# qurator-spk/sbb_textline_detection

Measured on AMD Instinct MI355X. Metric: segmented patches/sec (448x448x3) per GPU + per-pixel label-map match vs ref, higher is better.
Workload: dtype f16x3; 1 GPU; BASELINE configs[1] x 32: 32 pages of 3500x2500 (70 tiles of 448x448 each, margin 0.1) per GPU per step, textline model, 2 classes; workload_id=page, dedupe=False, max_batch=320, lanes=2, owned_regions=1, exchange=none

## Files before the change

sbb_textline_detection_amd/csrc/api.hip:

```cpp
#include <stdarg.h>
#include <stdio.h>
#include <stdlib.h>
#include <string.h>

#include <algorithm>
#include <cmath>
#include <new>
#include <stdexcept>
#include <string>
#include <utility>
#include <vector>

#include "../../include/sbbseg.h"
#include <dlfcn.h>

#include <mutex>

#include "internal.h"
#include "region.h"
#include "profile_stat.h"
#include "line_mask.h"
#include "line_split.h"

using namespace sbbseg;
// ... 139 lines not shown
    double prof_ms = 0;
    int64_t prof_launches = 0, prof_patches = 0;
    int region_level = -1;
    double exec_patches = 0;
    double prof_exec_patches = 0;
};

struct PendingEvent { int op; hipEvent_t a, b; int patches; double exec; };

struct RegionRun {
    bool on = false;
    int kind[kRegionMaxLevels] = {0};
    int total[kRegionMaxLevels] = {0};
    double frac[kRegionMaxLevels] = {0};
    uint32_t* tab[kRegionMaxLevels] = {nullptr};
};

}

struct sbbseg_ctx {
    int device = 0;
    int precision = kBF16;
    int elem = 2;
    int planes = 1;
    hipStream_t own_stream = nullptr;
    hipStream_t stream = nullptr;
    hipStream_t lane_stream = nullptr;
    hipEvent_t ev_fork = nullptr, ev_join = nullptr;
    int lanes = 2, lane1_batch = 0;
    int lane_prio = 0, prio_least = 0, prio_greatest = 0;
// ... 63 lines not shown
    bool block_pq = true;
    bool unfuse_blocks = false;
    bool unfuse_stem_pool = false;
    bool no_dec_halo = false;
    bool no_expand_reduce = false;
    bool no_c3er = false;
    bool plain_gather = false;
    int contig_max_k = 0;
    int fused_heads = 0;
    int num_cus = 256;
    std::vector<PendingEvent> pending;
    std::vector<hipEvent_t> free_events;
    int owned_mode = 1;
    int region_levels = 0;
    int region_op[kRegionMaxLevels] = {0};
    uint32_t* d_rtab[2][kRegionMaxLevels] = {{nullptr}, {nullptr}};
    size_t rtab_cap[2][kRegionMaxLevels] = {{0}, {0}};
    RegionRun rr;
    double last_exec_frac = 1.0;
    std::vector<std::pair<void*, size_t>> user_bufs;
};

namespace {

int dmalloc(sbbseg_ctx* c, void** p, size_t bytes)
{
    HIPCHK(hipMalloc(p, bytes));
    c->device_bytes += bytes;
    return 0;
}
// ... 177 lines not shown
            if (rlv >= 0 && c->rr.kind[rlv] == 1) {
                if (p.fast_gather && !p.half_stages && p.variant != 2 && !(p.variant_flags & 4)) { p.rmap = c->rr.tab[rlv]; p.M = c->rr.total[rlv]; }
                else c->last_exec_frac = 1.0;
            }
            if (co.d_stem_wfrag && !(c->conv_variant & 3)) {
                const Tensor& st = c->tensors[co.d.src[0].tensor];
                StemParams sp;
                sp.pairs = st.buf; sp.PHt = st.H; sp.PWt = st.W; sp.n = n; sp.Ho = co.Ho; sp.Wo = co.Wo;
                sp.wfrag = co.d_stem_wfrag; sp.scale = co.d_scale; sp.shift = co.d_shift; sp.relu = co.d.relu; sp.wmul = co.wmul_cls[0];
                sp.out = c->tensors[co.d.out_tensor].data();
                if (co.fused_pool >= 0 && !c->unfuse_stem_pool) {
                    const PoolOp& po = c->ops[co.fused_pool].pool;
                    sp.pool_out = c->tensors[po.dst].data(); sp.pool_scale = po.d_pre_scale; sp.pool_shift = po.d_pre_shift;
                    sp.pool_relu = po.pre_relu; sp.pool_Ho = po.Ho; sp.pool_Wo = po.Wo;
                    sp.x3 = c->precision == kF16X3;
                    HIPCHK(launch_stem_pool_x3(sp, c->num_cus, c->stream));
                } else
                    HIPCHK(launch_stem(sp, c->precision, c->num_cus, c->stream));
            } else if (co.d_d64_wfrag && !(c->conv_variant & 3)) {
                const Tensor& st = c->tensors[co.d.src[0].tensor];
                Direct64Params dp;
                dp.src = st.buf; dp.n = n; dp.H = st.H; dp.W = st.W; dp.wfrag = co.d_d64_wfrag;
                dp.scale = co.d_scale; dp.shift = co.d_shift; dp.relu = co.d.relu; dp.out = c->tensors[co.d.out_tensor].data();
                dp.wmul = co.wmul_cls[0];
                HIPCHK(launch_direct64(dp, c->precision, c->num_cus, c->stream));
            } else if (co.fused_reduce >= 0 && !c->no_expand_reduce && !(c->conv_variant & 3)) {
                const ConvOp& ro = c->ops[co.fused_reduce].conv;
                if (co.fused_conv3 >= 0 && !c->no_c3er) {
                    const ConvOp& k3 = c->ops[co.fused_conv3].conv;
                    const Tensor& ta = c->tensors[k3.d.src[0].tensor];
// ... 52 lines not shown
            }
        } else if (op.type == kPool) {
            const PoolOp& po = op.pool;
            if (po.fused_into_stem && !c->unfuse_stem_pool && !(c->conv_variant & 3)) return 0;
            const Tensor& s = c->tensors[po.src];
            HIPCHK(launch_maxpool(s.data(), c->tensors[po.dst].data(), n, s.H, s.W, s.C, po.k, po.stride, po.Ho, po.Wo,
                                  po.d_pre_scale, po.d_pre_shift, po.pre_relu, c->precision, c->stream));
        } else if (op.type == kTail) {
            const TailOp& to = op.tail;
            const Tensor& s0 = c->tensors[to.src0];
            TailParams tp;
            tp.src0 = s0.buf; tp.img = c->tensors[to.img].buf; tp.PH = s0.H; tp.PW = s0.W; tp.n = n;
            tp.wfrag = to.d_wfrag; tp.scale = to.d_scale; tp.shift = to.d_shift; tp.classes = to.classes;
            tp.head_w = to.d_head_w; tp.head_scale = to.d_head_scale; tp.head_shift = to.d_head_shift;
            tp.labels = d_labels; tp.probs = d_probs;
            if (c->rr.on && op.region_level >= 0) {
                if (c->rr.total[op.region_level] == 0) return 0;
                tp.ttab = c->rr.tab[op.region_level]; tp.n_tab = c->rr.total[op.region_level];
            }
            HIPCHK(launch_tail(tp, c->precision, c->num_cus, c->stream));
        } else {
            const HeadOp& ho = op.head;
            const Tensor& s = c->tensors[ho.src];
            HeadParams hp;
            hp.src = s.data(); hp.cin = ho.cin; hp.classes = ho.classes; hp.M = n * s.H * s.W;
            hp.w = ho.d_w; hp.scale = ho.d_scale; hp.shift = ho.d_shift;
            hp.labels = d_labels; hp.probs = d_probs;
            HIPCHK(launch_head(hp, c->precision, c->stream));
        }
    return 0;
// ... 294 lines not shown
        (void)hipFree(c->pp_d_in[k]); (void)hipFree(c->pp_d_out[k]); (void)hipFree(c->pp_d_out3[k]);
        if (c->pp_in[k]) (void)hipEventDestroy(c->pp_in[k]);
        if (c->pp_comp[k]) (void)hipEventDestroy(c->pp_comp[k]);
        if (c->pp_out[k]) (void)hipEventDestroy(c->pp_out[k]);
    }
    comm_release(c);
    if (c->copy_in) (void)hipStreamDestroy(c->copy_in);
    if (c->copy_out) (void)hipStreamDestroy(c->copy_out);
    (void)hipFree(c->d_morph_a); (void)hipFree(c->d_morph_b); (void)hipFree(c->d_cc_parent); (void)hipFree(c->d_cc_count); (void)hipFree(c->d_cc_aux); (void)hipFree(c->d_cc_list); (void)hipFree(c->d_cc_small);
    for (auto& pe : c->pending) { (void)hipEventDestroy(pe.a); (void)hipEventDestroy(pe.b); }
    for (auto e : c->free_events) (void)hipEventDestroy(e);
    if (c->own_stream) (void)hipStreamDestroy(c->own_stream);
    if (c->lane_stream) (void)hipStreamDestroy(c->lane_stream);
    if (c->ev_fork) (void)hipEventDestroy(c->ev_fork);
    if (c->ev_join) (void)hipEventDestroy(c->ev_join);
    delete c;
    return 0;
    API_END
}

int sbbseg_set_stream(sbbseg_ctx* c, void* hip_stream)
{
    API_BEGIN
    REQUIRE(c, "null handle");
    if (resolve_pending(c)) return 1;
    c->stream = hip_stream == SBBSEG_OWN_STREAM ? c->own_stream : (hipStream_t)hip_stream;
    int up = 0;
    if (hip_stream != SBBSEG_OWN_STREAM && hip_stream && c->lane_prio != 0 && c->prio_least != c->prio_greatest &&
        hipStreamGetPriority((hipStream_t)hip_stream, &up) == hipSuccess && up == c->lane_prio) {
        const int other = c->lane_prio == c->prio_greatest ? c->prio_least : c->prio_greatest;
// ... 1090 lines not shown
            Op& b = c->ops[i + 1];
            if (a.type != kConv || !a.conv.d_stem_wfrag || b.type != kPool) continue;
            const PoolOp& po = b.pool;
            const Tensor& f1 = c->tensors[a.conv.d.out_tensor];
            if (po.src != a.conv.d.out_tensor || po.k != 3 || po.stride != 2 || !po.d_pre_scale || f1.C != 64 || (f1.H & 15) || (f1.W & 15) ||
                po.Ho != f1.H / 2 - 1 || po.Wo != f1.W / 2 - 1)
                continue;
            a.conv.fused_pool = (int)(i + 1);
            b.pool.fused_into_stem = true;
        }
    }
    REQUIRE(max_batch >= 1, "max_batch must be >= 1");
    REQUIRE(c->classes > 0 && !c->ops.empty(), "plan must contain a head (head op or a conv with a fused head)");
    c->max_batch = max_batch;
    find_region_chain(c);
    for (auto& t : c->tensors) {
        const size_t bytes = kZeroHeaderBytes + t.elems_per_patch * max_batch * c->elem * c->planes + 256;
        REQUIRE(bytes < ((size_t)1 << 32), "tensor %dx%dx%d x batch %d exceeds the 4 GiB gather window", t.H, t.W, t.C, max_batch);
        if (dmalloc(c, (void**)&t.lane_buf[0], bytes)) return 1;
        t.buf = t.lane_buf[0];
        HIPCHK(hipMemset(t.buf, 0, t.is_input_form ? bytes : (size_t)kZeroHeaderBytes));
    }
    c->lane1_batch = (c->lanes == 2 && max_batch >= 2 * kMinLaneTiles) ? (max_batch + 1) / 2 : 0;
    if (c->lane1_batch)
        for (auto& t : c->tensors) {
            const size_t bytes = kZeroHeaderBytes + t.elems_per_patch * c->lane1_batch * c->elem * c->planes + 256;
            if (dmalloc(c, (void**)&t.lane_buf[1], bytes)) return 1;
            HIPCHK(hipMemset(t.lane_buf[1], 0, t.is_input_form ? bytes : (size_t)kZeroHeaderBytes));
        }
    for (const Op& op : c->ops)
// ... 163 lines not shown
{
    REQUIRE(d_pages && n_pages >= 1 && d_tile_labels && first_tile >= 0 && n_tiles >= 0, "bad arguments");
    for (int k = 0; k < n_pages; ++k) REQUIRE(d_pages[k], "null page pointer (page %d)", k);
    int nx = 0, ny = 0;
    if (fused_grid(c, Hp, Wp, dedupe, &nx, &ny)) return 1;
    const int tpp = nx * ny;
    REQUIRE((long)first_tile + n_tiles <= (long)tpp * n_pages, "tile range [%d,%d) exceeds the %d tiles of the %d page(s)", first_tile,
            first_tile + n_tiles, tpp * n_pages, n_pages);
    const int margin = margin_of(c->in_W);
    IngestParams ip;
    if (fill_ingest(c, ip)) return 1;
    ip.page = (const uint8_t*)d_pages[0]; ip.Hp = Hp; ip.Wp = Wp; ip.src_Hp = src_Hp; ip.src_Wp = src_Wp; ip.tile_xy = nullptr;
    ip.map_y = d_map_y; ip.map_x = d_map_x; ip.bin_thr = d_bin_thr;
    ip.grid_nyf = ny; ip.grid_mid_x = c->in_W - 2 * margin; ip.grid_mid_y = c->in_H - 2 * margin;
    const size_t per = (size_t)c->in_H * c->in_W;
    const size_t act = (size_t)c->elem * c->planes;
    const bool regions = owned && c->region_levels > 0 && c->max_batch <= kRegionMaxPatches;
    RegionGeom rg;
    memset(&rg, 0, sizeof(rg));
    if (regions) {
        rg.ax = {Wp, c->in_W, margin, c->in_W - 2 * margin, nx};
        rg.ay = {Hp, c->in_H, margin, c->in_H - 2 * margin, ny};
        rg.tpp = tpp; rg.ny = ny; rg.n_levels = c->region_levels;
        for (int L = 0; L < c->region_levels; ++L) {
            const Op& lop = c->ops[c->region_op[L]];
            if (L == 0) { rg.kind[L] = 0; rg.Rh[L] = c->in_H; rg.Rw[L] = c->in_W; rg.align_x[L] = 16; }
            else {
                const Tensor& to = c->tensors[lop.conv.d.out_tensor];
                rg.kind[L] = runs_dec_halo(c, lop.conv) ? 0 : 1;
                rg.Rh[L] = to.H; rg.Rw[L] = to.W; rg.align_x[L] = 2;
            }
// ... 12 lines not shown
                total += region_entries(rg, i, j, L);
            }
            const size_t need = 4 * (rg.kind[L] ? 4 * batch_cap * (size_t)(rg.Rh[L] / 2) * (size_t)(rg.Rw[L] / 2)
                                                 : batch_cap * (size_t)(rg.Rh[L] / 16 + 1) * (size_t)(rg.Rw[L] / 16 + 1));
            if (c->rtab_cap[lane][L] < need) {
                HIPCHK(hipDeviceSynchronize());
                if (c->d_rtab[lane][L]) { HIPCHK(hipFree(c->d_rtab[lane][L])); c->device_bytes -= c->rtab_cap[lane][L]; c->d_rtab[lane][L] = nullptr; c->rtab_cap[lane][L] = 0; }
                if (dmalloc(c, (void**)&c->d_rtab[lane][L], need)) return 1;
                c->rtab_cap[lane][L] = need;
            }
            bp.out[L] = c->d_rtab[lane][L]; bp.total[L] = (int)total;
            rr.kind[L] = rg.kind[L]; rr.total[L] = (int)total; rr.tab[L] = c->d_rtab[lane][L];
            rr.frac[L] = (double)total * (rg.kind[L] ? 4.0 : 256.0) / ((double)nb * rg.Rh[L] * rg.Rw[L]);
        }
        HIPCHK(launch_region_build(bp, c->stream));
        rr.on = true;
        return 0;
    };
    struct RegionOff { sbbseg_ctx* c; ~RegionOff() { c->rr.on = false; } };
    auto run_chunk = [&](int lane, int first, int nb) -> int {
        LaneScope scope(c, lane);
        RegionOff roff{c};
        if (regions && setup_regions(lane, first_tile + first, nb)) return 1;
        IngestParams lp = ip;
        if (fill_ingest(c, lp)) return 1;
        char* const c8_base = (char*)lp.c8;
        char* const pairs_base = (char*)lp.pairs;
        const size_t c8_tile = per * 8 * act, pairs_tile = lp.pairs ? (size_t)(c->in_H + 2 * lp.pad) * lp.pairs_w * 8 * act : 0;
        lp.Hp = ip.Hp; lp.Wp = ip.Wp; lp.src_Hp = ip.src_Hp; lp.src_Wp = ip.src_Wp; lp.tile_xy = nullptr;
        lp.map_y = ip.map_y; lp.map_x = ip.map_x; lp.bin_thr = ip.bin_thr;
        lp.grid_nyf = ip.grid_nyf; lp.grid_mid_x = ip.grid_mid_x; lp.grid_mid_y = ip.grid_mid_y;
        for (int done = 0; done < nb;) {
            const int g = first_tile + first + done, pg = g / tpp, local = g - pg * tpp;
            const int run = nb - done < tpp - local ? nb - done : tpp - local;
            lp.page = (const uint8_t*)d_pages[pg];
            lp.grid_first = local;
            lp.n_tiles = run;
            lp.c8 = c8_base + (size_t)done * c8_tile;
            lp.pairs = pairs_base ? pairs_base + (size_t)done * pairs_tile : nullptr;
            HIPCHK(launch_ingest_u8(lp, c->precision, c->stream));
            done += run;
        }
        return run_plan(c, nb, (uint8_t*)d_tile_labels + first * per, nullptr);
    };
    const int chunk_cap = (c->profiling && c->lanes == 2 && c->lane1_batch > 0 && c->max_batch >= 4 * kMinLaneTiles) ? (c->max_batch + 1) / 2 : c->max_batch;
    const int n_chunks = (n_tiles + chunk_cap - 1) / chunk_cap;
    const int chunk = n_chunks ? (n_tiles + n_chunks - 1) / n_chunks : 0;
    bool forked = false;
    for (int done = 0; done < n_tiles; done += chunk) {
        const int nb = n_tiles - done < chunk ? n_tiles - done : chunk;
        const bool two = c->lane1_batch > 0 && c->lanes == 2 && !c->profiling && nb >= 2 * kMinLaneTiles;
        if (!two) {
            if (forked) {
                HIPCHK(hipEventRecord(c->ev_join, c->lane_stream));
                HIPCHK(hipStreamWaitEvent(c->stream, c->ev_join, 0));
                forked = false;
            }
// ... 1763 lines not shown
```

sbb_textline_detection_amd/csrc/internal.h:

```cpp
#pragma once
#include <hip/hip_runtime.h>
#include <stdint.h>

namespace sbbseg {

constexpr int kZeroHeaderBytes = 256;
constexpr int kBK = 64;
constexpr int kGranulesPerStep = 8;

struct SrcDesc {
    const char* base;
    int PH, PW;
    int pix_bytes;
    int shift;
    int lim_y, lim_x;
    int ksteps;
    int sy_shift, sx_shift;
    int lo_off;
    uint32_t bytes;
    int tap_lo_y, tap_lo_x;
};

struct KTabEntry {
    int16_t dy, dx;
// ... 52 lines not shown
    const float* head_shift;
    uint8_t* labels;
    float* probs;
    uint32_t howo_magic, howo_shift, wo_magic, wo_shift, nct_magic, nct_shift;
    const FgStepRec* fgstep_cls[4];
    int fast_gather;
    int ks_shift;
    float* ks_ws;
    long ks_split_elems;
    const uint32_t* rmap;
};

struct TailParams {
    const char* src0;
    const char* img;
    int PH, PW;
    int n;
    const void* wfrag;
    const float* scale;
    const float* shift;
    int classes;
    const float* head_w;
    const float* head_scale;
    const float* head_shift;
    uint8_t* labels;
    float* probs;
    const uint32_t* ttab = nullptr;
    int n_tab = 0;
};

struct StemParams {
    const char* pairs;
    int PHt, PWt;
    int n;
    int Ho, Wo;
    const void* wfrag;
    const float* scale;
    const float* shift;
    int relu;
    float wmul;
    void* out;
    void* pool_out = nullptr;
    const float* pool_scale = nullptr;
    const float* pool_shift = nullptr;
    int pool_relu = 0;
    int pool_Ho = 0, pool_Wo = 0;
    int x3 = 1;
};

struct Direct64Params {
    const char* src;
    int n, H, W;
    const void* wfrag;
    const float* scale;
    const float* shift;
    int relu;
    float wmul;
    void* out;
};

#if defined(__HIPCC__)
#define SBBSEG_HD __host__ __device__
// ... 74 lines not shown

struct HeadParams {
    const void* src;
    int cin;
    int classes;
    int M;
    const float* w;
    const float* scale;
    const float* shift;
    uint8_t* labels;
    float* probs;
};

struct IngestParams {
    const uint8_t* page;
    int Hp, Wp;
    int src_Hp, src_Wp;
    int whole;
    const int* tile_xy;
    int grid_first, grid_nyf;
    int grid_mid_x, grid_mid_y;
    int n_tiles;
    int H, W;
    const float* lut;
    void* c8;
    void* pairs;
    int pad, pairs_w;
    const int* map_y;
    const int* map_x;
    const int* bin_thr;
// ... 148 lines not shown
```

sbb_textline_detection_amd/csrc/kernels.hip:

```cpp
#include "internal.h"

namespace sbbseg {

typedef __attribute__((ext_vector_type(8))) short bf16x8_t;
typedef __attribute__((ext_vector_type(8))) _Float16 f16x8_t;
typedef __attribute__((ext_vector_type(2))) _Float16 f16x2_t;
typedef __attribute__((ext_vector_type(4))) float f32x4_t;

#define GLOBAL_AS __attribute__((address_space(1)))
#define LDS_AS __attribute__((address_space(3)))

__host__ __device__ inline uint16_t bf16_bits_rne(float f)
{
    uint32_t u = __builtin_bit_cast(uint32_t, f);
    if ((u & 0x7fffffffu) > 0x7f800000u) return (uint16_t)((u >> 16) | 0x40);
    u += 0x7fffu + ((u >> 16) & 1u);
    return (uint16_t)(u >> 16);
}
uint16_t f32_to_bf16_rne(float f) { return bf16_bits_rne(f); }
float bf16_to_f32(uint16_t h) { uint32_t u = (uint32_t)h << 16; return __builtin_bit_cast(float, u); }
uint16_t f32_to_f16_rne(float f)
{
    f = f > 65504.f ? 65504.f : (f < -65504.f ? -65504.f : f);
    _Float16 h = (_Float16)f;
// ... 1470 lines not shown
        __syncthreads();
        if (tid < 16)
            *(uint4*)(p.labels + (size_t)(n * H + ty0 + tid) * W + tx0) = *(const uint4*)(lbl_tile + tid * 16);
    }
}

constexpr int kT3SrcBytes = 10 * 16 * 256;
constexpr int kT3ImgBytes = 18 * 32 * 16;
constexpr int kT3BufBytes = kT3SrcBytes + kT3ImgBytes;
constexpr int kT3HalfSteps = 10;

constexpr int kT3PsPartBytes = 2 * 4 * 64 * 4 * 4;
constexpr int kT3PsLdsBytes = 2 * kT3BufBytes + 2 * 256 + kTailConstBytes + kT3PsPartBytes;
static_assert(kT3PsLdsBytes <= 160 * 1024, "x3 tail: LDS");

template <int NC>
__global__ __launch_bounds__(512, 2) void dec_tail_fused_x3ps(const TailParams p)
{
    constexpr bool F16 = true;
    extern __shared__ __attribute__((aligned(16))) char smem[];
    char* lbl_tile = smem + 2 * kT3BufBytes;
    float* cst = (float*)(lbl_tile + 2 * 256);
    float* part = (float*)((char*)cst + kTailConstBytes);

    const int tid = threadIdx.x;
    const int lane = tid & 63;
    const int wave = __builtin_amdgcn_readfirstlane(tid >> 6);
    const int par = wave & 3, mh = wave >> 2;
    const int py = par >> 1, px = par & 1;
    const int frow = lane & 15, fg = lane >> 4;

// ... 51 lines not shown
    float hsc[NC], hsh[NC];
#pragma unroll
    for (int c = 0; c < NC; ++c) { hsc[c] = c < p.classes ? p.head_scale[c] : 0.f; hsh[c] = c < p.classes ? p.head_shift[c] : 0.f; }

    const int hp0 = ((frow >> 3) + py) * 16 + (frow & 7) + px;
    const int s0 = (fg + 2 * hp0) & 15;
    int src_t[8];
#pragma unroll
    for (int e = 0; e < 8; ++e) src_t[e] = hp0 * 256 + (((s0 + 2 * e) & 15) << 4);
    int img_t[3];
#pragma unroll
    for (int e = 0; e < 3; ++e) {
        const int t0 = (e >> 1) * 8 + 2 * fg + (e & 1);
        const int t = t0 < 9 ? t0 : 1;
        const int yb = 2 * (frow >> 3) + py + t / 3, x = 2 * (frow & 7) + px + t % 3;
        img_t[e] = yb * 512 + ((((x >> 1) + 12 * (x & 1) + 16 - 4 * (yb & 3)) & 31) << 4);
    }

    const int c_src = par * 4 + (lane >> 4);
    const uint32_t voff_src = (uint32_t)(c_src * 256 + ((((lane & 15) - 2 * c_src) & 15) << 4));
    const int img_v = ((lane & 31) - (16 - 4 * ((2 * par + (lane >> 5)) & 3))) & 31;
    const bool img_xok = img_v < 9 || (img_v >= 12 && img_v < 21);
    const int img_x = img_v < 9 ? 2 * img_v : 2 * (img_v - 12) + 1;
    const uint32_t voff_img = (uint32_t)(((lane >> 5) * W + img_x) * 32);
    const uint32_t src_img_bytes = (uint32_t)(p.PH * p.PW) * 256u, img_img_bytes = (uint32_t)(H * W) * 32u;
    auto issue_src = [&](int n, int y0, int x0, int buf) __attribute__((always_inline)) {
        char* lds_src = smem + buf * kT3BufBytes;
        const char* sbase = p.src0 + kZeroHeaderBytes - 256 + (size_t)n * src_img_bytes;
        const uint32_t vs = ((unsigned)((x0 >> 1) - 1 + c_src) < (unsigned)p.PW && c_src < 10) ? voff_src : 0x80000000u;
#pragma unroll
        for (int j = 0; j < 10; ++j) {
            const int Y = (y0 >> 1) - 1 + j;
            const bool yok = (unsigned)Y < (unsigned)p.PH;
            const uint32_t soff = yok ? (uint32_t)(Y * p.PW + (x0 >> 1)) * 256u : 0u;
            buffer_load_lds16(sbase, src_img_bytes + 256u, (LDS_AS void*)(lds_src + (par + 4 * j) * 1024), yok ? vs : 0x80000000u, soff);
        }
    };
    auto issue_img = [&](int n, int y0, int x0, int buf) __attribute__((always_inline)) {
        char* lds_img = smem + buf * kT3BufBytes + kT3SrcBytes;
        const char* ibase = p.img + kZeroHeaderBytes + (size_t)n * img_img_bytes - (size_t)(W + 1) * 32;
        const uint32_t vi = (img_xok && (unsigned)(x0 - 1 + img_x) < (unsigned)W) ? voff_img : 0x80000000u;
#pragma unroll
        for (int j = 0; j < 3; ++j) {
            const int q = par + 4 * j;
            if (q < 9) {
                const bool yok = (unsigned)(y0 - 1 + 2 * q + (lane >> 5)) < (unsigned)H;
                buffer_load_lds16(ibase, img_img_bytes + (uint32_t)(W + 1) * 32u, (LDS_AS void*)(lds_img + q * 1024), yok ? vi : 0x80000000u,
                                  (uint32_t)((y0 + 2 * q) * W + x0) * 32u);
            }
        }
    };

    f32x4_t acc[4];
    auto main_loop = [&](int it) __attribute__((always_inline)) {
// ... 5 lines not shown
#pragma unroll
        for (int e = 0; e < 8; ++e) sb[e] = lds_src + src_t[e];
        auto load_b = [&](int h, bf16x8_t (&bh)[4], bf16x8_t (&bl)[4]) __attribute__((always_inline)) {
            if (h < 8) {
                const int ks = h >> 1, kk = h & 1;
                const int dh = (kk * 8 + 2 * (ks & 1)) & 15, dl = (kk * 8 + 4 + 2 * (ks & 1)) & 15;
#pragma unroll
                for (int ni = 0; ni < 4; ++ni) {
                    const int k = (ni * 32 + (ks >> 1) * 16 + (ks & 1)) * 256;
                    bh[ni] = *(const bf16x8_t*)(sb[dh >> 1] + k);
                    bl[ni] = *(const bf16x8_t*)(sb[dl >> 1] + k);
                }
            } else {
#pragma unroll
                for (int ni = 0; ni < 4; ++ni) {
                    const uint4 r0 = *(const uint4*)(lds_img + img_t[(h - 8) * 2] + ni * 2048);
                    const uint4 r1 = h == 8 ? *(const uint4*)(lds_img + img_t[1] + ni * 2048) : r0;
                    bh[ni] = __builtin_bit_cast(bf16x8_t, make_uint4(r0.x, r0.y, r1.x, r1.y));
                    bl[ni] = __builtin_bit_cast(bf16x8_t, make_uint4(r0.z, r0.w, r1.z, r1.w));
                }
            }
        };
        auto mac = [&](int h, const bf16x8_t (&bh)[4], const bf16x8_t (&bl)[4]) __attribute__((always_inline)) {
#pragma unroll
            for (int ni = 0; ni < 4; ++ni) acc[ni] = mfma16<F16>(wlo[h], bh[ni], acc[ni]);
#pragma unroll
            for (int ni = 0; ni < 4; ++ni) acc[ni] = mfma16<F16>(whi[h], bl[ni], acc[ni]);
#pragma unroll
            for (int ni = 0; ni < 4; ++ni) acc[ni] = mfma16<F16>(whi[h], bh[ni], acc[ni]);
        };
        bf16x8_t b0h[4], b0l[4], b1h[4], b1l[4];
        load_b(0, b0h, b0l);
#pragma unroll
        for (int h = 0; h < NH; h += 2) {
// ... 117 lines not shown
    auto go = [&](auto kern) -> hipError_t {
        hipError_t e = hipFuncSetAttribute((const void*)kern, hipFuncAttributeMaxDynamicSharedMemorySize, kTailLdsBytes);
        if (e != hipSuccess) return e;
        hipLaunchKernelGGL(kern, dim3(grid), dim3(256), kTailLdsBytes, s, p);
        return hipSuccess;
    };
    hipError_t e;
    if (precision == kF16X3) {
        const int grid3 = ((n_tiles < num_cus ? n_tiles : num_cus) + 7) & ~7;
        auto gops = [&](auto kern) -> hipError_t {
            hipError_t e8 = hipFuncSetAttribute((const void*)kern, hipFuncAttributeMaxDynamicSharedMemorySize, kT3PsLdsBytes);
            if (e8 != hipSuccess) return e8;
            hipLaunchKernelGGL(kern, dim3(grid3), dim3(512), kT3PsLdsBytes, s, p);
            return hipSuccess;
        };
        e = p.classes <= 2 ? gops(dec_tail_fused_x3ps<2>) : gops(dec_tail_fused_x3ps<4>);
        if (e != hipSuccess) return e;
        return hipGetLastError();
    }
    if (precision == kF16) e = p.classes <= 2 ? go(dec_tail_fused<true, 2>) : go(dec_tail_fused<true, 4>);
    else e = p.classes <= 2 ? go(dec_tail_fused<false, 2>) : go(dec_tail_fused<false, 4>);
    if (e != hipSuccess) return e;
    return hipGetLastError();
}

constexpr int kStemRowSlots = 20;
constexpr int kStemRows = 37;
constexpr int kStemInstr = (kStemRows * kStemRowSlots + 63) / 64;
constexpr int kStemBufBytes = kStemInstr * 1024;
constexpr int kStemLdsBytes = 2 * kStemBufBytes + 512;
constexpr int kStemStores = 8;
// ... 1069 lines not shown
template <typename E> struct alignas(sizeof(E) * 4) Vec4 { E v[4]; };

template <typename E>
__device__ inline void write_split_input(const float (&f)[3], void* c8, void* pairs, long idx, int t, int y, int x,
                                         int H, int pad, int pairs_w)
{
    _Float16 hi[3], lo[3];
#pragma unroll
    for (int i = 0; i < 3; ++i) split_f32(f[i], hi[i], lo[i]);
    const _Float16 z = (_Float16)0.f;
    Vec8<_Float16> oh, ol;
#pragma unroll
    for (int i = 0; i < 8; ++i) { oh.v[i] = i < 3 ? hi[i] : z; ol.v[i] = i < 3 ? lo[i] : z; }
#pragma unroll
    for (int i = 0; i < 3; ++i) oh.v[4 + i] = lo[i];
    ((Vec8<_Float16>*)c8)[2 * idx] = oh;
    ((Vec8<_Float16>*)c8)[2 * idx + 1] = ol;
    if (pairs) {
        const int PH = H + 2 * pad;
        const int xp = x + pad;
        _Float16* dst = (_Float16*)pairs + (((size_t)t * PH + (y + pad)) * pairs_w + (xp >> 1)) * 16 + (xp & 1) * 4;
        Vec4<_Float16> qh, ql;
        qh.v[0] = hi[0]; qh.v[1] = hi[1]; qh.v[2] = hi[2]; qh.v[3] = z;
        ql.v[0] = lo[0]; ql.v[1] = lo[1]; ql.v[2] = lo[2]; ql.v[3] = z;
        *(Vec4<_Float16>*)dst = qh;
        *(Vec4<_Float16>*)(dst + 8) = ql;
    }
}

template <typename E, bool SPLIT = false>
__global__ __launch_bounds__(256) void ingest_u8_kernel(const IngestParams p)
{
    const long idx = (long)blockIdx.x * 256 + threadIdx.x;
    const long per = (long)p.H * p.W;
    if (idx >= per * p.n_tiles) return;
    const int t = (int)(idx / per);
    const int rem = (int)(idx - t * per);
    const int y = rem / p.W, x = rem - y * p.W;
    int vy, vx;
    if (p.whole) { vy = y; vx = x; }
    else if (p.tile_xy) { vx = p.tile_xy[2 * t] + x; vy = p.tile_xy[2 * t + 1] + y; }
    else {
        const int gt = p.grid_first + t;
        const int gi = gt / p.grid_nyf, gj = gt - gi * p.grid_nyf;
        vx = min(gi * p.grid_mid_x, p.Wp - p.W) + x;
        vy = min(gj * p.grid_mid_y, p.Hp - p.H) + y;
    }
    const int sy = p.map_y ? p.map_y[vy] : vy, sx = p.map_x ? p.map_x[vx] : vx;
    const uint8_t* px = p.page + ((size_t)sy * p.src_Wp + sx) * 3;
    E v0, v1, v2;
    if (p.bin_thr) {
        v0 = v1 = v2 = to_elem<E>((int)px[0] > *p.bin_thr ? 1.f : 0.f);
    } else {
        v0 = to_elem<E>(p.lut[px[0]]); v1 = to_elem<E>(p.lut[px[1]]); v2 = to_elem<E>(p.lut[px[2]]);
    }
    const E z = to_elem<E>(0.f);
    if constexpr (SPLIT) {
        float f[3];
        if (p.bin_thr) f[0] = f[1] = f[2] = (int)px[0] > *p.bin_thr ? 1.f : 0.f;
        else { f[0] = p.lut[px[0]]; f[1] = p.lut[px[1]]; f[2] = p.lut[px[2]]; }
        write_split_input<E>(f, p.c8, p.pairs, idx, t, y, x, p.H, p.pad, p.pairs_w);
        return;
    }
    Vec8<E> o;
    o.v[0] = v0; o.v[1] = v1; o.v[2] = v2;
#pragma unroll
    for (int i = 3; i < 8; ++i) o.v[i] = z;
    ((Vec8<E>*)p.c8)[idx] = o;
    if (p.pairs) {
        const int PH = p.H + 2 * p.pad;
        const int xp = x + p.pad;
        E* dst = (E*)p.pairs + (((size_t)t * PH + (y + p.pad)) * p.pairs_w + (xp >> 1)) * 8 + (xp & 1) * 4;
        Vec4<E> q; q.v[0] = v0; q.v[1] = v1; q.v[2] = v2; q.v[3] = z;
        *(Vec4<E>*)dst = q;
    }
}

template <typename E, bool SPLIT = false>
__global__ __launch_bounds__(256) void ingest_f32_kernel(const float* x, int n, int H, int W, void* c8,
                                                         void* pairs, int pad, int pairs_w)
{
    const long idx = (long)blockIdx.x * 256 + threadIdx.x;
    const long per = (long)H * W;
// ... 845 lines not shown
```

sbb_textline_detection_amd/csrc/region.h:

```cpp
#pragma once
#include "internal.h"

namespace sbbseg {

constexpr int kRegionMaxLevels = 8;

struct RegionAxis {
    int extent, tile, margin, mid, n;
};

struct RegionGeom {
    RegionAxis ax, ay;
    int tpp, ny;
    int n_levels;
    int kind[kRegionMaxLevels];
    int Rh[kRegionMaxLevels], Rw[kRegionMaxLevels];
    int align_x[kRegionMaxLevels];
};

SBBSEG_HD inline int region_origin(const RegionAxis& a, int t) { return t * a.mid + a.tile > a.extent ? a.extent - a.tile : t * a.mid; }

SBBSEG_HD inline void region_own(const RegionAxis& a, int t, int& lo, int& hi)
{
    const int o = region_origin(a, t);
    lo = t == 0 ? 0 : a.margin;
    hi = t == a.n - 1 ? a.tile : a.tile - a.margin;
    if (t + 1 < a.n) {
        const int cut = region_origin(a, t + 1) + a.margin - o;
        if (cut < hi) hi = cut;
    }
    if (hi < lo) hi = lo;
}

// ... 28 lines not shown
    const int o = (lo & ~(align - 1)) + 16 * k;
    return o + 16 > R ? R - 16 : o;
}

SBBSEG_HD inline int region_entries(const RegionGeom& g, int i, int j, int level)
{
    int ylo, yhi, xlo, xhi;
    region_needed(g, i, j, level, ylo, yhi, xlo, xhi);
    if (yhi <= ylo) return 0;
    if (g.kind[level] == 0) return region_tiles16(ylo, yhi, 2) * region_tiles16(xlo, xhi, g.align_x[level]);
    region_even(ylo, yhi, g.Rh[level]);
    region_even(xlo, xhi, g.Rw[level]);
    return ((yhi - ylo) >> 1) * ((xhi - xlo) >> 1);
}

SBBSEG_HD inline uint32_t region_code(int n, int y, int x) { return ((uint32_t)n << 22) | ((uint32_t)y << 11) | (uint32_t)x; }
SBBSEG_HD inline int region_code_n(uint32_t c) { return (int)(c >> 22); }
SBBSEG_HD inline int region_code_y(uint32_t c) { return (int)((c >> 11) & 2047u); }
SBBSEG_HD inline int region_code_x(uint32_t c) { return (int)(c & 2047u); }
constexpr int kRegionMaxPatches = 1023, kRegionMaxCoord = 2047;

struct RegionBuildParams {
    RegionGeom g;
    int g0, nb;
    uint32_t* out[kRegionMaxLevels];
    int total[kRegionMaxLevels];
};
hipError_t launch_region_build(const RegionBuildParams& p, hipStream_t s);

}
// ... 1 lines not shown
```

sbb_textline_detection_amd/csrc/stem_pool_x3.hip:

```cpp
#include "internal.h"

namespace sbbseg {

namespace {

typedef __attribute__((ext_vector_type(8))) _Float16 h8_t;
typedef __attribute__((ext_vector_type(4))) float f4_t;

constexpr int kSlots = 20;
constexpr int kHaloRows = 39;
constexpr int kHaloInstr = (kHaloRows * kSlots + 63) / 64;
constexpr int kPlaneBytes = kHaloInstr * 1024;
constexpr int kColStride = 36;
constexpr int kStageVBytes = 8 * 18 * kColStride * 4;
constexpr int kStageRBytes = 5 * 16 * kColStride * 4;
constexpr int kSaveBytes = 2 * 8 * 2 * kColStride * 4;
constexpr int kCstBytes = 4 * 64 * 4;
constexpr int kWloBytes = 7 * 2 * 1024;
constexpr int kStemPoolLdsBytes = 2 * kPlaneBytes + kStageVBytes + kStageRBytes + kSaveBytes + kCstBytes + kWloBytes;
constexpr int kStemPoolF16LdsBytes = kPlaneBytes + kStageVBytes + kStageRBytes + kSaveBytes + kCstBytes;

__device__ inline f4_t mma(h8_t a, h8_t b, f4_t c) { return __builtin_amdgcn_mfma_f32_16x16x32_f16(a, b, c, 0, 0, 0); }

__device__ inline void glds16_hidden(const void* gsrc, uint32_t lds_dst)
// ... 59 lines not shown
#pragma unroll
            for (int j = 0; j < (kHaloInstr + 3) / 4; ++j) {
                const int ii = wave + 4 * j;
                if (ii < kHaloInstr) {
                    const int s = ii * 64 + lane;
                    const int r = s / kSlots, cc = s - r * kSlots;
                    const int Y = 32 * ty + r, X = 16 * tx + cc;
                    uint32_t off = (uint32_t)((n * p.PHt + Y) * p.PWt + X) * (uint32_t)(16 * NPL) + (uint32_t)(pl * 16 + kZeroHeaderBytes);
                    off = r < rows ? off : 0u;
                    glds16_hidden(p.pairs + off, halo_lds + (uint32_t)(pl * kPlaneBytes + ii * 1024));
                }
            }
    };

    int first = 1;
    int par = 0;
    for (int strip = slot * 8 + xcd; strip < n_strips; strip += n_slots * 8) {
        const int n = strip / tiles_y, ty = strip - n * tiles_y;
        const bool last_ty = ty == tiles_y - 1;
        for (int tx = 0; tx < tiles_x; ++tx) {
            if (first) { issue_halo(n, ty, tx); first = 0; asm volatile("s_waitcnt vmcnt(0)" ::: "memory"); }
            else if constexpr (X3) asm volatile("s_waitcnt vmcnt(8)" ::: "memory");
            else asm volatile("s_waitcnt vmcnt(4)" ::: "memory");
            asm volatile("s_waitcnt lgkmcnt(0)" ::: "memory");
            __builtin_amdgcn_s_barrier();
            asm volatile("" ::: "memory");

            f4_t acc[2][4], accx[2] = {(f4_t){0.f, 0.f, 0.f, 0.f}, (f4_t){0.f, 0.f, 0.f, 0.f}};
#pragma unroll
            for (int m = 0; m < 2; ++m)
#pragma unroll
                for (int ni = 0; ni < 4; ++ni) acc[m][ni] = (f4_t){0.f, 0.f, 0.f, 0.f};
            {
                h8_t bh[2], bl[2], wlo[2][2];
                auto frag = [&](int step, h8_t& dh, h8_t& dl) __attribute__((always_inline)) {
                    const int ky = step >> 2, ni = step & 3;
                    const int at = ((2 * (wave * 4 + ni) + ky) * kSlots + frow + fg) * 16;
                    dh = *(const h8_t*)(halo + at);
                    if constexpr (X3) dl = *(const h8_t*)(halo + kPlaneBytes + at);
                };
                auto wfrag = [&](int ky, h8_t (&d)[2]) __attribute__((always_inline)) {
                    if constexpr (X3) {
// ... 55 lines not shown
#pragma unroll
                    for (int q = 0; q < 8; ++q) {
                        float y = __builtin_fmaf(acc[q >> 2][ni][q & 3], sc[q], sh[q]);
                        if (p.relu) y = fmaxf(y, 0.f);
                        if constexpr (X3) {
                            _Float16 a, b;
                            split1(y, a, b);
                            vh[q] = a; vl[q] = b;
                            acc[q >> 2][ni][q & 3] = __fadd_rn((float)a, (float)b);
                        } else {
                            vh[q] = (_Float16)__builtin_amdgcn_fmed3f(y, -65504.f, 65504.f);
                            acc[q >> 2][ni][q & 3] = (float)vh[q];
                        }
                    }
                    if constexpr (X3) {
                        uint16_t* dst = (uint16_t*)p.out + pix * 128 + half * 64 + fg * 8;
                        *(h8_t*)dst = vh;
                        *(h8_t*)(dst + 32) = vl;
                    } else {
                        *(h8_t*)((uint16_t*)p.out + pix * 64 + half * 32 + fg * 8) = vh;
                    }
                }
            }
            __builtin_amdgcn_sched_barrier(0);
            {
                float ps[8], pb[8];
                *(float4*)&ps[0] = *(const float4*)(cst + 128 + c0); *(float4*)&ps[4] = *(const float4*)(cst + 128 + c0 + 4);
                *(float4*)&pb[0] = *(const float4*)(cst + 192 + c0); *(float4*)&pb[4] = *(const float4*)(cst + 192 + c0 + 4);
                float v0[8], v1[8];
#pragma unroll
                for (int ni = 0; ni < 4; ++ni) {
                    float zz[8];
#pragma unroll
// ... 131 lines not shown
```

Before: 5693 patches/s.

## Skip unused stem/c8 stores, read pairs in tail, single multi-page ingest launch

Three changes land together. The stem+pool x3 kernel now skips writing full-resolution stem outputs outside the region later consumed via a skip connection, which cuts write traffic. The tail kernel reads the padded pairs input tensor instead of the c8 image tensor, so the ingest can skip writing c8 when nothing else reads it. The per-page loop of ingest launches is also replaced by one launch driven by a device-side page-pointer table uploaded through pinned memory. Together these add complexity, an event sync on the pointer buffer, and correctness risk when the stem skip-region geometry is computed wrongly.

```diff
diff --git a/sbb_textline_detection_amd/csrc/api.hip b/sbb_textline_detection_amd/csrc/api.hip
--- a/sbb_textline_detection_amd/csrc/api.hip
+++ b/sbb_textline_detection_amd/csrc/api.hip
@@ -177,6 +177,8 @@
     int total[kRegionMaxLevels] = {0};
     double frac[kRegionMaxLevels] = {0};
     uint32_t* tab[kRegionMaxLevels] = {nullptr};
+    RegionGeom geom = {};
+    int g0 = 0;
 };
 
 }
@@ -270,6 +272,11 @@
     int owned_mode = 1;
     int region_levels = 0;
     int region_op[kRegionMaxLevels] = {0};
+    bool tail_pairs = false, page_c8 = true;
+    const void** d_page_ptrs = nullptr; size_t page_ptrs_cap = 0;
+    const void** h_page_ptrs = nullptr; size_t h_page_ptrs_cap = 0;
+    hipEvent_t ev_ptrs = nullptr;
+    int stem_skip_level = -1;
     uint32_t* d_rtab[2][kRegionMaxLevels] = {{nullptr}, {nullptr}};
     size_t rtab_cap[2][kRegionMaxLevels] = {{0}, {0}};
     RegionRun rr;
@@ -477,6 +484,10 @@
                     sp.pool_out = c->tensors[po.dst].data(); sp.pool_scale = po.d_pre_scale; sp.pool_shift = po.d_pre_shift;
                     sp.pool_relu = po.pre_relu; sp.pool_Ho = po.Ho; sp.pool_Wo = po.Wo;
                     sp.x3 = c->precision == kF16X3;
+                    if (c->rr.on && sp.x3 && c->stem_skip_level >= 0) {
+                        sp.rg_on = 1; sp.rg = c->rr.geom; sp.rg_g0 = c->rr.g0; sp.rg_level = c->stem_skip_level;
+                        sp.rg.kind[sp.rg_level] = c->rr.kind[sp.rg_level];
+                    }
                     HIPCHK(launch_stem_pool_x3(sp, c->num_cus, c->stream));
                 } else
                     HIPCHK(launch_stem(sp, c->precision, c->num_cus, c->stream));
@@ -559,6 +570,10 @@
             tp.wfrag = to.d_wfrag; tp.scale = to.d_scale; tp.shift = to.d_shift; tp.classes = to.classes;
             tp.head_w = to.d_head_w; tp.head_scale = to.d_head_scale; tp.head_shift = to.d_head_shift;
             tp.labels = d_labels; tp.probs = d_probs;
+            if (c->tail_pairs) {
+                const Tensor& pr = c->tensors[c->form_tensor[SBBSEG_INPUT_PAIRS]];
+                tp.img = pr.buf; tp.img_pairs = 1; tp.img_PHt = pr.H; tp.img_PWt = pr.W; tp.img_pad = pr.pad;
+            }
             if (c->rr.on && op.region_level >= 0) {
                 if (c->rr.total[op.region_level] == 0) return 0;
                 tp.ttab = c->rr.tab[op.region_level]; tp.n_tab = c->rr.total[op.region_level];
@@ -883,6 +898,8 @@
     if (c->lane_stream) (void)hipStreamDestroy(c->lane_stream);
     if (c->ev_fork) (void)hipEventDestroy(c->ev_fork);
     if (c->ev_join) (void)hipEventDestroy(c->ev_join);
+    if (c->ev_ptrs) (void)hipEventDestroy(c->ev_ptrs);
+    (void)hipFree(c->d_page_ptrs); (void)hipHostFree(c->h_page_ptrs);
     delete c;
     return 0;
     API_END
@@ -2003,6 +2020,47 @@
     REQUIRE(c->classes > 0 && !c->ops.empty(), "plan must contain a head (head op or a conv with a fused head)");
     c->max_batch = max_batch;
     find_region_chain(c);
+    {
+        const char* envfb = getenv("SBBSEG_FUSE_BLOCKS");
+        const int c8t = c->form_tensor[SBBSEG_INPUT_C8], prt = c->form_tensor[SBBSEG_INPUT_PAIRS];
+        c->tail_pairs = c->precision == kF16X3 && c->ops.back().type == kTail && c->ops.back().tail.img == c8t && prt >= 0 && c->tensors[prt].pad >= 2;
+        int c8_readers = 0;
+        for (size_t k = 0; k < c->ops.size(); ++k) {
+            const Op& o = c->ops[k];
+            auto conv_reads = [&](const ConvOp& co) { for (int q = 0; q < co.d.n_src; ++q) c8_readers += co.d.src[q].tensor == c8t; c8_readers += co.d.residual_tensor == c8t; };
+            if (o.type == kConv) conv_reads(o.conv);
+            else if (o.type == kPool) c8_readers += o.pool.src == c8t;
+            else if (o.type == kHead) c8_readers += o.head.src == c8t;
+            else if (o.type == kTail) c8_readers += (o.tail.src0 == c8t) + (o.tail.img == c8t && !(c->tail_pairs && k + 1 == c->ops.size()));
+            else if (o.type == kBlock) { c8_readers += o.block.x_tensor == c8t; for (const Op& q : o.parts) if (q.type == kConv) conv_reads(q.conv); }
+        }
+        if (c->tail_pairs)
+            c->ops.back().min_bytes -= (double)c->in_H * c->in_W * (8 * c->elem * c->planes - 16);
+        c->page_c8 = c8_readers > 0 || prt < 0 || (envfb && envfb[0] == '0');
+    }
+    c->stem_skip_level = -1;
+    for (size_t i = 0; i < c->ops.size(); ++i) {
+        const Op& a = c->ops[i];
+        if (a.type != kConv || a.conv.fused_pool < 0) continue;
+        const int f1 = a.conv.d.out_tensor;
+        int level = -1, others = 0;
+        for (size_t k = 0; k < c->ops.size(); ++k) {
+            const Op& o = c->ops[k];
+            if ((int)k == a.conv.fused_pool) { others += o.pool.src != f1; continue; }
+            if (o.type == kConv) {
+                const sbbseg_conv_desc& d = o.conv.d;
+                const bool skip_src = o.region_level >= 1 && d.n_src == 2 && d.src[1].tensor == f1 && d.src[0].tensor != f1 && d.residual_tensor != f1 &&
+                                      c->tensors[f1].H == c->tensors[d.out_tensor].H && c->tensors[f1].W == c->tensors[d.out_tensor].W;
+                if (skip_src && level < 0) { level = o.region_level; continue; }
+                for (int q = 0; q < d.n_src; ++q) others += d.src[q].tensor == f1;
+                others += d.residual_tensor == f1;
+            } else if (o.type == kPool) others += o.pool.src == f1;
+            else if (o.type == kHead) others += o.head.src == f1;
+            else if (o.type == kTail) others += (o.tail.src0 == f1) + (o.tail.img == f1);
+            else if (o.type == kBlock) others += o.block.x_tensor == f1;
+        }
+        if (level >= 1 && others == 0) c->stem_skip_level = level;
+    }
     for (auto& t : c->tensors) {
         const size_t bytes = kZeroHeaderBytes + t.elems_per_patch * max_batch * c->elem * c->planes + 256;
         REQUIRE(bytes < ((size_t)1 << 32), "tensor %dx%dx%d x batch %d exceeds the 4 GiB gather window", t.H, t.W, t.C, max_batch);
@@ -2196,7 +2254,21 @@
     ip.map_y = d_map_y; ip.map_x = d_map_x; ip.bin_thr = d_bin_thr;
     ip.grid_nyf = ny; ip.grid_mid_x = c->in_W - 2 * margin; ip.grid_mid_y = c->in_H - 2 * margin;
     const size_t per = (size_t)c->in_H * c->in_W;
-    const size_t act = (size_t)c->elem * c->planes;
+    if (n_pages > 1) {
+        const size_t bytes = sizeof(void*) * (size_t)n_pages;
+        if (ensure(c, (void**)&c->d_page_ptrs, &c->page_ptrs_cap, bytes)) return 1;
+        if (!c->ev_ptrs) HIPCHK(hipEventCreateWithFlags(&c->ev_ptrs, hipEventDisableTiming));
+        else HIPCHK(hipEventSynchronize(c->ev_ptrs));
+        if (c->h_page_ptrs_cap < bytes) {
+            if (c->h_page_ptrs) { HIPCHK(hipHostFree(c->h_page_ptrs)); c->h_page_ptrs = nullptr; c->h_page_ptrs_cap = 0; }
+            HIPCHK(hipHostMalloc((void**)&c->h_page_ptrs, bytes, hipHostMallocDefault));
+            c->h_page_ptrs_cap = bytes;
+        }
+        memcpy(c->h_page_ptrs, d_pages, bytes);
+        HIPCHK(hipMemcpyAsync(c->d_page_ptrs, c->h_page_ptrs, bytes, hipMemcpyHostToDevice, c->stream));
+        HIPCHK(hipEventRecord(c->ev_ptrs, c->stream));
+        ip.pages = (const uint8_t* const*)c->d_page_ptrs; ip.tpp = tpp;
+    }
     const bool regions = owned && c->region_levels > 0 && c->max_batch <= kRegionMaxPatches;
     RegionGeom rg;
     memset(&rg, 0, sizeof(rg));
@@ -2239,6 +2311,7 @@
             rr.frac[L] = (double)total * (rg.kind[L] ? 4.0 : 256.0) / ((double)nb * rg.Rh[L] * rg.Rw[L]);
         }
         HIPCHK(launch_region_build(bp, c->stream));
+        rr.geom = rg; rr.g0 = g_first;
         rr.on = true;
         return 0;
     };
@@ -2249,23 +2322,14 @@
         if (regions && setup_regions(lane, first_tile + first, nb)) return 1;
         IngestParams lp = ip;
         if (fill_ingest(c, lp)) return 1;
-        char* const c8_base = (char*)lp.c8;
-        char* const pairs_base = (char*)lp.pairs;
-        const size_t c8_tile = per * 8 * act, pairs_tile = lp.pairs ? (size_t)(c->in_H + 2 * lp.pad) * lp.pairs_w * 8 * act : 0;
+        if (!c->page_c8) lp.c8 = nullptr;
+        lp.page = ip.page; lp.pages = ip.pages; lp.tpp = ip.tpp;
         lp.Hp = ip.Hp; lp.Wp = ip.Wp; lp.src_Hp = ip.src_Hp; lp.src_Wp = ip.src_Wp; lp.tile_xy = nullptr;
         lp.map_y = ip.map_y; lp.map_x = ip.map_x; lp.bin_thr = ip.bin_thr;
         lp.grid_nyf = ip.grid_nyf; lp.grid_mid_x = ip.grid_mid_x; lp.grid_mid_y = ip.grid_mid_y;
-        for (int done = 0; done < nb;) {
-            const int g = first_tile + first + done, pg = g / tpp, local = g - pg * tpp;
-            const int run = nb - done < tpp - local ? nb - done : tpp - local;
-            lp.page = (const uint8_t*)d_pages[pg];
-            lp.grid_first = local;
-            lp.n_tiles = run;
-            lp.c8 = c8_base + (size_t)done * c8_tile;
-            lp.pairs = pairs_base ? pairs_base + (size_t)done * pairs_tile : nullptr;
-            HIPCHK(launch_ingest_u8(lp, c->precision, c->stream));
-            done += run;
-        }
+        lp.grid_first = first_tile + first;
+        lp.n_tiles = nb;
+        if (nb > 0) HIPCHK(launch_ingest_u8(lp, c->precision, c->stream));
         return run_plan(c, nb, (uint8_t*)d_tile_labels + first * per, nullptr);
     };
     const int chunk_cap = (c->profiling && c->lanes == 2 && c->lane1_batch > 0 && c->max_batch >= 4 * kMinLaneTiles) ? (c->max_batch + 1) / 2 : c->max_batch;
diff --git a/sbb_textline_detection_amd/csrc/internal.h b/sbb_textline_detection_amd/csrc/internal.h
--- a/sbb_textline_detection_amd/csrc/internal.h
+++ b/sbb_textline_detection_amd/csrc/internal.h
@@ -90,6 +90,7 @@
 struct TailParams {
     const char* src0;
     const char* img;
+    int img_pairs = 0, img_PHt = 0, img_PWt = 0, img_pad = 0;
     int PH, PW;
     int n;
     const void* wfrag;
@@ -103,6 +104,21 @@
     float* probs;
     const uint32_t* ttab = nullptr;
     int n_tab = 0;
+};
+
+constexpr int kRegionMaxLevels = 8;
+
+struct RegionAxis {
+    int extent, tile, margin, mid, n;
+};
+
+struct RegionGeom {
+    RegionAxis ax, ay;
+    int tpp, ny;
+    int n_levels;
+    int kind[kRegionMaxLevels];
+    int Rh[kRegionMaxLevels], Rw[kRegionMaxLevels];
+    int align_x[kRegionMaxLevels];
 };
 
 struct StemParams {
@@ -122,6 +138,8 @@
     int pool_relu = 0;
     int pool_Ho = 0, pool_Wo = 0;
     int x3 = 1;
+    int rg_on = 0, rg_g0 = 0, rg_level = 0;
+    RegionGeom rg = {};
 };
 
 struct Direct64Params {
@@ -226,6 +244,8 @@
 
 struct IngestParams {
     const uint8_t* page;
+    const uint8_t* const* pages;
+    int tpp;
     int Hp, Wp;
     int src_Hp, src_Wp;
     int whole;
diff --git a/sbb_textline_detection_amd/csrc/kernels.hip b/sbb_textline_detection_amd/csrc/kernels.hip
--- a/sbb_textline_detection_amd/csrc/kernels.hip
+++ b/sbb_textline_detection_amd/csrc/kernels.hip
@@ -1508,7 +1508,7 @@
 constexpr int kT3PsLdsBytes = 2 * kT3BufBytes + 2 * 256 + kTailConstBytes + kT3PsPartBytes;
 static_assert(kT3PsLdsBytes <= 160 * 1024, "x3 tail: LDS");
 
-template <int NC>
+template <int NC, bool PAIRS>
 __global__ __launch_bounds__(512, 2) void dec_tail_fused_x3ps(const TailParams p)
 {
     constexpr bool F16 = true;
@@ -1590,8 +1590,13 @@
         const int t0 = (e >> 1) * 8 + 2 * fg + (e & 1);
         const int t = t0 < 9 ? t0 : 1;
         const int yb = 2 * (frow >> 3) + py + t / 3, x = 2 * (frow & 7) + px + t % 3;
+        if constexpr (PAIRS) {
+            const int xg = x + ((p.img_pad - 1) & 1);
+            img_t[e] = yb * 512 + ((((xg >> 1) + 4 * (yb & 3)) & 15) << 4) + (xg & 1) * 8;
+        } else
         img_t[e] = yb * 512 + ((((x >> 1) + 12 * (x & 1) + 16 - 4 * (yb & 3)) & 31) << 4);
     }
+
 
     const int c_src = par * 4 + (lane >> 4);
     const uint32_t voff_src = (uint32_t)(c_src * 256 + ((((lane & 15) - 2 * c_src) & 15) << 4));
@@ -1600,6 +1605,9 @@
     const int img_x = img_v < 9 ? 2 * img_v : 2 * (img_v - 12) + 1;
     const uint32_t voff_img = (uint32_t)(((lane >> 5) * W + img_x) * 32);
     const uint32_t src_img_bytes = (uint32_t)(p.PH * p.PW) * 256u, img_img_bytes = (uint32_t)(H * W) * 32u;
+    const int pr_g = ((lane & 15) - 4 * ((2 * par + (lane >> 5)) & 3)) & 15;
+    const uint32_t pr_voff = pr_g < 10 ? (uint32_t)(((lane >> 5) * p.img_PWt + pr_g) * 32 + ((lane >> 4) & 1) * 16) : 0x80000000u;
+    const uint32_t pr_img_bytes = (uint32_t)(p.img_PHt * p.img_PWt) * 32u;
     auto issue_src = [&](int n, int y0, int x0, int buf) __attribute__((always_inline)) {
         char* lds_src = smem + buf * kT3BufBytes;
         const char* sbase = p.src0 + kZeroHeaderBytes - 256 + (size_t)n * src_img_bytes;
@@ -1614,6 +1622,17 @@
     };
     auto issue_img = [&](int n, int y0, int x0, int buf) __attribute__((always_inline)) {
         char* lds_img = smem + buf * kT3BufBytes + kT3SrcBytes;
+        if constexpr (PAIRS) {
+            const char* pbase = p.img + kZeroHeaderBytes + (size_t)n * pr_img_bytes;
+#pragma unroll
+            for (int j = 0; j < 3; ++j) {
+                const int q = par + 4 * j;
+                if (q < 9)
+                    buffer_load_lds16(pbase, pr_img_bytes, (LDS_AS void*)(lds_img + q * 1024), pr_voff,
+                                      (uint32_t)((y0 - 1 + p.img_pad + 2 * q) * p.img_PWt + ((x0 - 1 + p.img_pad) >> 1)) * 32u);
+            }
+            return;
+        }
         const char* ibase = p.img + kZeroHeaderBytes + (size_t)n * img_img_bytes - (size_t)(W + 1) * 32;
         const uint32_t vi = (img_xok && (unsigned)(x0 - 1 + img_x) < (unsigned)W) ? voff_img : 0x80000000u;
 #pragma unroll
@@ -1649,10 +1668,20 @@
             } else {
 #pragma unroll
                 for (int ni = 0; ni < 4; ++ni) {
+                    if constexpr (PAIRS) {
+                        auto rd = [](const char* a) __attribute__((always_inline)) { uint2 v; v.x = 0; v.y = 0; const unsigned long long q = *(const volatile LDS_AS unsigned long long*)a; v.x = (uint32_t)q; v.y = (uint32_t)(q >> 32); return v; };
+                        const char* a0 = lds_img + img_t[(h - 8) * 2] + ni * 2048;
+                        const char* a1 = lds_img + img_t[1] + ni * 2048;
+                        const uint2 h0 = rd(a0), l0 = rd(a0 + 256);
+                        const uint2 h1 = h == 8 ? rd(a1) : h0, l1 = h == 8 ? rd(a1 + 256) : l0;
+                        bh[ni] = __builtin_bit_cast(bf16x8_t, make_uint4(h0.x, h0.y, h1.x, h1.y));
+                        bl[ni] = __builtin_bit_cast(bf16x8_t, make_uint4(l0.x, l0.y, l1.x, l1.y));
+                    } else {
                     const uint4 r0 = *(const uint4*)(lds_img + img_t[(h - 8) * 2] + ni * 2048);
                     const uint4 r1 = h == 8 ? *(const uint4*)(lds_img + img_t[1] + ni * 2048) : r0;
                     bh[ni] = __builtin_bit_cast(bf16x8_t, make_uint4(r0.x, r0.y, r1.x, r1.y));
                     bl[ni] = __builtin_bit_cast(bf16x8_t, make_uint4(r0.z, r0.w, r1.z, r1.w));
+                    }
                 }
             }
         };
@@ -1800,7 +1829,8 @@
             hipLaunchKernelGGL(kern, dim3(grid3), dim3(512), kT3PsLdsBytes, s, p);
             return hipSuccess;
         };
-        e = p.classes <= 2 ? gops(dec_tail_fused_x3ps<2>) : gops(dec_tail_fused_x3ps<4>);
+        if (p.img_pairs) e = p.classes <= 2 ? gops(dec_tail_fused_x3ps<2, true>) : gops(dec_tail_fused_x3ps<4, true>);
+        else e = p.classes <= 2 ? gops(dec_tail_fused_x3ps<2, false>) : gops(dec_tail_fused_x3ps<4, false>);
         if (e != hipSuccess) return e;
         return hipGetLastError();
     }
@@ -2900,8 +2930,10 @@
     for (int i = 0; i < 8; ++i) { oh.v[i] = i < 3 ? hi[i] : z; ol.v[i] = i < 3 ? lo[i] : z; }
 #pragma unroll
     for (int i = 0; i < 3; ++i) oh.v[4 + i] = lo[i];
-    ((Vec8<_Float16>*)c8)[2 * idx] = oh;
-    ((Vec8<_Float16>*)c8)[2 * idx + 1] = ol;
+    if (c8) {
+        ((Vec8<_Float16>*)c8)[2 * idx] = oh;
+        ((Vec8<_Float16>*)c8)[2 * idx + 1] = ol;
+    }
     if (pairs) {
         const int PH = H + 2 * pad;
         const int xp = x + pad;
@@ -2927,13 +2959,18 @@
     if (p.whole) { vy = y; vx = x; }
     else if (p.tile_xy) { vx = p.tile_xy[2 * t] + x; vy = p.tile_xy[2 * t + 1] + y; }
     else {
-        const int gt = p.grid_first + t;
+        const int gt = p.pages ? (p.grid_first + t) % p.tpp : p.grid_first + t;
         const int gi = gt / p.grid_nyf, gj = gt - gi * p.grid_nyf;
         vx = min(gi * p.grid_mid_x, p.Wp - p.W) + x;
         vy = min(gj * p.grid_mid_y, p.Hp - p.H) + y;
     }
     const int sy = p.map_y ? p.map_y[vy] : vy, sx = p.map_x ? p.map_x[vx] : vx;
-    const uint8_t* px = p.page + ((size_t)sy * p.src_Wp + sx) * 3;
+    const uint8_t* page = p.page;
+    if (p.pages) {
+        const int g = p.grid_first + t;
+        page = p.pages[g / p.tpp];
+    }
+    const uint8_t* px = page + ((size_t)sy * p.src_Wp + sx) * 3;
     E v0, v1, v2;
     if (p.bin_thr) {
         v0 = v1 = v2 = to_elem<E>((int)px[0] > *p.bin_thr ? 1.f : 0.f);
@@ -2952,7 +2989,7 @@
     o.v[0] = v0; o.v[1] = v1; o.v[2] = v2;
 #pragma unroll
     for (int i = 3; i < 8; ++i) o.v[i] = z;
-    ((Vec8<E>*)p.c8)[idx] = o;
+    if (p.c8) ((Vec8<E>*)p.c8)[idx] = o;
     if (p.pairs) {
         const int PH = p.H + 2 * p.pad;
         const int xp = x + p.pad;
diff --git a/sbb_textline_detection_amd/csrc/region.h b/sbb_textline_detection_amd/csrc/region.h
--- a/sbb_textline_detection_amd/csrc/region.h
+++ b/sbb_textline_detection_amd/csrc/region.h
@@ -3,20 +3,6 @@
 
 namespace sbbseg {
 
-constexpr int kRegionMaxLevels = 8;
-
-struct RegionAxis {
-    int extent, tile, margin, mid, n;
-};
-
-struct RegionGeom {
-    RegionAxis ax, ay;
-    int tpp, ny;
-    int n_levels;
-    int kind[kRegionMaxLevels];
-    int Rh[kRegionMaxLevels], Rw[kRegionMaxLevels];
-    int align_x[kRegionMaxLevels];
-};
 
 SBBSEG_HD inline int region_origin(const RegionAxis& a, int t) { return t * a.mid + a.tile > a.extent ? a.extent - a.tile : t * a.mid; }
 
@@ -75,6 +61,24 @@
     return ((yhi - ylo) >> 1) * ((xhi - xlo) >> 1);
 }
 
+SBBSEG_HD inline void region_skip_rect(const RegionGeom& g, int i, int j, int level, int& y0, int& y1, int& x0, int& x1)
+{
+    int ylo, yhi, xlo, xhi;
+    region_needed(g, i, j, level, ylo, yhi, xlo, xhi);
+    if (yhi <= ylo) { y0 = y1 = x0 = x1 = 0; return; }
+    if (g.kind[level] == 0) {
+        const int ax = g.align_x[level];
+        y0 = region_tile_origin(ylo, 2, 0, g.Rh[level]) - 1;
+        y1 = region_tile_origin(ylo, 2, region_tiles16(ylo, yhi, 2) - 1, g.Rh[level]) + 17;
+        x0 = region_tile_origin(xlo, ax, 0, g.Rw[level]) - 1;
+        x1 = region_tile_origin(xlo, ax, region_tiles16(xlo, xhi, ax) - 1, g.Rw[level]) + 17;
+    } else {
+        region_even(ylo, yhi, g.Rh[level]);
+        region_even(xlo, xhi, g.Rw[level]);
+        y0 = ylo - 1; y1 = yhi + 1; x0 = xlo - 1; x1 = xhi + 1;
+    }
+}
+
 SBBSEG_HD inline uint32_t region_code(int n, int y, int x) { return ((uint32_t)n << 22) | ((uint32_t)y << 11) | (uint32_t)x; }
 SBBSEG_HD inline int region_code_n(uint32_t c) { return (int)(c >> 22); }
 SBBSEG_HD inline int region_code_y(uint32_t c) { return (int)((c >> 11) & 2047u); }
diff --git a/sbb_textline_detection_amd/csrc/stem_pool_x3.hip b/sbb_textline_detection_amd/csrc/stem_pool_x3.hip
--- a/sbb_textline_detection_amd/csrc/stem_pool_x3.hip
+++ b/sbb_textline_detection_amd/csrc/stem_pool_x3.hip
@@ -1,4 +1,5 @@
 #include "internal.h"
+#include "region.h"
 
 namespace sbbseg {
 
@@ -97,18 +98,29 @@
     };
 
     int first = 1;
+    bool stored = true;
     int par = 0;
     for (int strip = slot * 8 + xcd; strip < n_strips; strip += n_slots * 8) {
         const int n = strip / tiles_y, ty = strip - n * tiles_y;
         const bool last_ty = ty == tiles_y - 1;
+        int st_x0 = 0, st_x1 = p.Wo;
+        if constexpr (X3) {
+            if (p.rg_on) {
+                const int local = (p.rg_g0 + n) % p.rg.tpp, gi = local / p.rg.ny, gj = local - gi * p.rg.ny;
+                int ry0, ry1;
+                region_skip_rect(p.rg, gi, gj, p.rg_level, ry0, ry1, st_x0, st_x1);
+                if (16 * ty >= ry1 || 16 * ty + 16 <= ry0) st_x0 = st_x1 = 0;
+            }
+        }
         for (int tx = 0; tx < tiles_x; ++tx) {
-            if (first) { issue_halo(n, ty, tx); first = 0; asm volatile("s_waitcnt vmcnt(0)" ::: "memory"); }
+            if (first || !stored) { if (first) issue_halo(n, ty, tx); first = 0; asm volatile("s_waitcnt vmcnt(0)" ::: "memory"); }
             else if constexpr (X3) asm volatile("s_waitcnt vmcnt(8)" ::: "memory");
             else asm volatile("s_waitcnt vmcnt(4)" ::: "memory");
             asm volatile("s_waitcnt lgkmcnt(0)" ::: "memory");
             __builtin_amdgcn_s_barrier();
             asm volatile("" ::: "memory");
 
+            stored = !X3 || (16 * tx < st_x1 && 16 * tx + 16 > st_x0);
             f4_t acc[2][4], accx[2] = {(f4_t){0.f, 0.f, 0.f, 0.f}, (f4_t){0.f, 0.f, 0.f, 0.f}};
 #pragma unroll
             for (int m = 0; m < 2; ++m)
@@ -194,9 +206,11 @@
                         }
                     }
                     if constexpr (X3) {
-                        uint16_t* dst = (uint16_t*)p.out + pix * 128 + half * 64 + fg * 8;
-                        *(h8_t*)dst = vh;
-                        *(h8_t*)(dst + 32) = vl;
+                        if (stored) {
+                            uint16_t* dst = (uint16_t*)p.out + pix * 128 + half * 64 + fg * 8;
+                            *(h8_t*)dst = vh;
+                            *(h8_t*)(dst + 32) = vl;
+                        }
                     } else {
                         *(h8_t*)((uint16_t*)p.out + pix * 64 + half * 32 + fg * 8) = vh;
                     }
```

Result: no change. 5723 patches/s, median of 6 (+0.5%).
